# oraclefina/MSPI

Hardware: AMD Instinct MI355X
Metric: clips_per_sec (higher is better)
Workload: dtype f32 storage/accumulate; GEMMs as f16x3 split products on the f16 MFMA pipe; 1 GPU; x3dl motion encoder + ConvNeXt-T + ResNet18 audio + SyncBlock + decoder (AudioVisualSaliencyModel forward), batch 8/GPU, clips 3x16x224x224, spectrogram 1x257x300, inputs resident in HBM; global_batch=8, launch=hipGraph replay (mspi_amd.runtime.GraphPipeline), 2 batches in flight, stream_layout=2, parallelism=single GPU

## Files before the change

include/mspi_hip.h:

```cpp
#ifndef MSPI_HIP_H
#define MSPI_HIP_H

#include <stddef.h>
#include <stdint.h>

#ifdef __cplusplus
extern "C" {
#endif

#define MSPI_ABI_VERSION 2

typedef void* mspi_stream_t;

enum {
  MSPI_OK = 0,
  MSPI_EINVAL = -1,
  MSPI_ELAUNCH = -2,
  MSPI_ENODEV = -3
};

enum { MSPI_ACT_NONE = 0, MSPI_ACT_RELU = 1, MSPI_ACT_GELU = 2, MSPI_ACT_SIGMOID = 3, MSPI_ACT_SWISH = 4 };

enum { MSPI_PREC_F32 = 0, MSPI_PREC_F16X3 = 1 };

// ... 79 lines not shown
int mspi_attn_fwd_ws(const MspiAttnDesc* d, const float* q, const float* k, const float* v, const float* res,
                     const float* biasT, const float* maskT, const int32_t* tok_idx, float* o, void* workspace,
                     mspi_stream_t stream);
int mspi_attn_variant(const MspiAttnDesc* d, int32_t has_bias, int32_t has_mask, int32_t has_tok, int32_t has_ws);

typedef struct MspiMvitAugDesc {
  int32_t B, heads, Dh, DA;
  int32_t qT, qH, qW, kT, kH, kW;
  int64_t ldq, ldk;
  float scale;
} MspiMvitAugDesc;

int mspi_mvit_qk_augment(const MspiMvitAugDesc* d, const float* q, const float* k, const float* Rh, const float* Rw,
                         const float* Rt, float* qa, float* ka, mspi_stream_t stream);

int mspi_mvit_qk_augment_p(const MspiMvitAugDesc* d, const float* q, const float* k, const float* P, int64_t ldp,
                           const int32_t* idx_h, const int32_t* idx_w, const int32_t* idx_t, float* qa, float* ka,
                           mspi_stream_t stream);

typedef struct MspiX3dAbDesc {
  int32_t N, T, H, W;
  int32_t Cin, Cmid;
  int64_t ldx, ldu;
  int32_t act;
  float wa_scale;
} MspiX3dAbDesc;

int mspi_x3d_ab_supported(const MspiX3dAbDesc* d);
int mspi_x3d_ab_pool_rows(const MspiX3dAbDesc* d);
size_t mspi_x3d_ab_packed_bytes(int32_t Cin, int32_t Cmid);
int mspi_x3d_ab_fwd(const MspiX3dAbDesc* d, const void* x, const void* wa_packed, const void* bias_a, const void* wb,
                    const void* bias_b, void* u, void* pool , mspi_stream_t stream);
int mspi_x3d_ab_variant(const MspiX3dAbDesc* d);

int mspi_maxpool_fwd(const MspiDwConvDesc* d, const float* x, float* y, mspi_stream_t stream);

int mspi_upsample_fwd(const float* src, int64_t lds, float* dst, int64_t ldd, int32_t NT, int32_t H,
                      int32_t W, int32_t C, int32_t factor, int32_t accumulate, int32_t act,
                      mspi_stream_t stream);

int mspi_upsample_sum_fwd(const float* const* srcs, const int64_t* lds, const int32_t* factors, int32_t J, float* dst,
                          int64_t ldd, int32_t NT, int32_t Ho, int32_t Wo, int32_t C, int32_t accumulate, int32_t act,
                          mspi_stream_t stream);

int mspi_space_to_depth(const float* x, int64_t ldx, float* y, int64_t ldy, int32_t NT, int32_t H, int32_t W,
                        int32_t C, mspi_stream_t stream);

int mspi_rowgate(float* x, int64_t ldx, const float* mask, int64_t M, int32_t C, mspi_stream_t stream);

int mspi_logsumexp_sub(float* x, int32_t N, int32_t L, mspi_stream_t stream);

int mspi_mean_rows(const float* x, int64_t ldx, int64_t rows_per_sample_stride, float* out, int32_t N,
                   int32_t R, int32_t C, mspi_stream_t stream);

int mspi_mean_rows_slices(int32_t R);
int mspi_mean_rows_ws(const float* x, int64_t ldx, int64_t rows_per_sample_stride, float* out, float* ws, int32_t N,
                      int32_t R, int32_t C, mspi_stream_t stream);

int mspi_neg_cosine(const float* p, const float* z, float* out, int32_t N, int32_t C, float scale,
                    int32_t accumulate, mspi_stream_t stream);

size_t mspi_postprocess_workspace(int32_t N, int32_t H, int32_t W, int32_t Ho, int32_t Wo);
int mspi_postprocess_u8(const float* logmap, unsigned char* out, void* workspace, int32_t N, int32_t H, int32_t W,
                        int32_t Ho, int32_t Wo, mspi_stream_t stream);

typedef struct MspiJpegDesc {
// ... 149 lines not shown
```

mspi_amd/_lib.py:

```python
import ctypes as C
import os

_HERE = os.path.dirname(os.path.abspath(__file__))
LIB_PATH = os.environ.get("MSPI_LIB_PATH") or os.path.join(_HERE, "csrc", "libmspi_hip.so")

ACT_NONE, ACT_RELU, ACT_GELU, ACT_SIGMOID, ACT_SWISH = range(5)
PREC_F32, PREC_F16X3 = 0, 1


class MspiError(RuntimeError):
    pass


class ConvDesc(C.Structure):
    _fields_ = [
        ("N", C.c_int32), ("T", C.c_int32), ("H", C.c_int32), ("W", C.c_int32), ("C", C.c_int32),
        ("sN", C.c_int64), ("sT", C.c_int64), ("sH", C.c_int64), ("sW", C.c_int64), ("sC", C.c_int64),
        ("kT", C.c_int32), ("kH", C.c_int32), ("kW", C.c_int32),
        ("strT", C.c_int32), ("strH", C.c_int32), ("strW", C.c_int32),
        ("padT", C.c_int32), ("padH", C.c_int32), ("padW", C.c_int32),
        ("To", C.c_int32), ("Ho", C.c_int32), ("Wo", C.c_int32),
        ("Cout", C.c_int32),
        ("ldy", C.c_int64), ("ldw", C.c_int64), ("ldr", C.c_int64),
        ("act", C.c_int32),
# ... 38 lines not shown


class MlpDesc(C.Structure):
    _fields_ = [
        ("M", C.c_int64), ("C", C.c_int32), ("hidden", C.c_int32),
        ("ldx", C.c_int64), ("ldr", C.c_int64), ("ldy", C.c_int64),
        ("ln", C.c_int32), ("act", C.c_int32), ("eps", C.c_float),
        ("w1_scale", C.c_float), ("w2_scale", C.c_float),
    ]


class RowGemmDesc(C.Structure):
    _fields_ = [
        ("M", C.c_int64), ("K", C.c_int32), ("N", C.c_int32),
        ("ldx", C.c_int64), ("ldr", C.c_int64), ("ldy", C.c_int64), ("ldg", C.c_int64),
        ("act", C.c_int32), ("rows_per_sample", C.c_int32), ("w_scale", C.c_float),
    ]


class X3dCaDesc(C.Structure):
    _fields_ = [
        ("M", C.c_int64), ("D", C.c_int32), ("Cx", C.c_int32),
        ("ldu", C.c_int64), ("ldr", C.c_int64), ("ldy", C.c_int64), ("ldt", C.c_int64), ("ldg", C.c_int64),
        ("rows_per_sample", C.c_int32), ("wc_scale", C.c_float), ("wa_scale", C.c_float),
    ]


class X3dAbDesc(C.Structure):
    _fields_ = [
        ("N", C.c_int32), ("T", C.c_int32), ("H", C.c_int32), ("W", C.c_int32),
        ("Cin", C.c_int32), ("Cmid", C.c_int32),
        ("ldx", C.c_int64), ("ldu", C.c_int64),
        ("act", C.c_int32), ("wa_scale", C.c_float),
    ]


class PermuteDesc(C.Structure):
    _fields_ = [("dims", C.c_int32 * 6), ("strides", C.c_int64 * 6), ("src_elems", C.c_int64)]


class JpegDesc(C.Structure):
    _fields_ = [
        ("B", C.c_int32), ("H", C.c_int32), ("W", C.c_int32), ("quality", C.c_int32),
        ("pitch", C.c_int64), ("map_stride", C.c_int64), ("file_stride", C.c_int64), ("cap", C.c_int64),
        ("div", C.c_uint16 * 64),
        ("header", C.c_void_p), ("header_len", C.c_int32),
    ]


class JpegDecTables(C.Structure):
    _fields_ = [
        ("scan_len", C.c_int32), ("reserved", C.c_int32),
        ("quant", (C.c_uint16 * 64) * 3),
        ("comp_dc", C.c_uint8 * 4), ("comp_ac", C.c_uint8 * 4),
        ("counts", (C.c_uint8 * 16) * 4),
        ("vals", (C.c_uint8 * 256) * 4),
    ]


class JpegDecInfo(C.Structure):
    _fields_ = [
        ("H", C.c_int32), ("W", C.c_int32), ("ncomp", C.c_int32), ("hs", C.c_int32), ("vs", C.c_int32),
        ("scan_off", C.c_int32), ("scan_len", C.c_int32), ("reserved", C.c_int32),
        ("tables", JpegDecTables),
    ]

# ... 53 lines not shown
    "mspi_logspec_fwd": (C.c_int, [_P, C.c_int64, _P, _P, C.c_int32, _P, _P, C.c_int32, _P]),
    "mspi_resize_norm_fwd": (C.c_int, [_P, C.c_int32, C.c_int32, _P, _P, C.c_int64, C.c_int32, C.c_int32, _P, _P, C.c_int32,
                                        _P, _P, C.c_int32, _P, _P, _P]),
    "mspi_clip_resize_plan": (C.c_int, [_P, C.c_int32, C.c_int32, C.c_int32, C.c_int32, C.c_int32, _P]),
    "mspi_clip_resize_norm_fwd": (C.c_int, [_P, C.c_int32, C.c_int32, C.c_int32, _P, _P, _P, C.c_int32, C.c_int32, C.c_int64,
                                             C.c_int64, C.c_int64, C.c_int64, C.c_int32, C.c_int32, _P, _P, _P, C.c_int32, _P, _P,
                                             _P, C.c_int32, _P, _P, _P]),
    "mspi_layernorm_sp_fwd": (C.c_int, [_P, C.c_int64, C.c_int64, _P, C.c_int64, C.c_int64, _P, _P, C.c_float, C.c_int32,
                                         C.c_int32, C.c_int32, C.c_int32, _P]),
    "mspi_split_planes_fwd": (C.c_int, [_P, C.c_int64, C.c_int64, C.c_int32, _P, C.c_int64, C.c_int64, _P]),
    "mspi_join_planes_fwd": (C.c_int, [_P, C.c_int64, C.c_int64, C.c_int64, C.c_int32, _P, C.c_int64, _P]),
    "mspi_gemm_sp_fwd": (C.c_int, [C.POINTER(ConvDesc), _P, C.c_int64, C.c_int64, _P, _P, _P, _P, _P, C.c_int64, C.c_int64, _P]),
    "mspi_gemm_sp_variant": (C.c_int, [C.POINTER(ConvDesc), _P]),
    "mspi_saliency_metrics": (C.c_int, [_P, _P, _P, _P, C.c_int32, C.c_int32, C.c_int32, _P]),
    "mspi_saliency_auc_ws_bytes": (C.c_size_t, [C.c_int32, C.c_int32]),
    "mspi_saliency_auc_judd": (C.c_int, [_P, C.c_int32, _P, _P, _P, _P, C.c_int32, C.c_int32, _P]),
    "mspi_saliency_sauc_counts": (C.c_int, [_P, _P, _P, _P, C.c_int32, C.c_int32, C.c_int32, _P]),
    "mspi_saliency_ig": (C.c_int, [_P, _P, _P, _P, C.c_int32, C.c_int32, _P]),
    "mspi_resize_bilinear_fwd": (C.c_int, [_P, C.c_int32, _P, C.c_int32, C.c_int32, C.c_int32, C.c_int32, C.c_int32, _P]),
    "mspi_resize_fixation_fwd": (C.c_int, [_P, _P, C.c_int32, C.c_int32, C.c_int32, C.c_int32, C.c_int32, _P]),
    "mspi_rowgemm_packed_bytes": (C.c_size_t, [C.c_int32, C.c_int32]),
    "mspi_rowgemm_supported": (C.c_int, [C.c_int32, C.c_int32]),
    "mspi_rowgemm_fwd": (C.c_int, [C.POINTER(RowGemmDesc), _P, _P, _P, _P, _P, _P, _P]),
    "mspi_rowgemm_variant": (C.c_int, [C.POINTER(RowGemmDesc), C.c_int32]),
    "mspi_x3d_ca_packed_bytes": (C.c_size_t, [C.c_int32, C.c_int32]),
    "mspi_x3d_ca_supported": (C.c_int, [C.c_int32, C.c_int32]),
    "mspi_x3d_ca_fwd": (C.c_int, [C.POINTER(X3dCaDesc), _P, _P, _P, _P, _P, _P, _P, _P, _P]),
    "mspi_x3d_ca_variant": (C.c_int, [C.POINTER(X3dCaDesc), C.c_int32]),
    "mspi_x3d_ab_supported": (C.c_int, [C.POINTER(X3dAbDesc)]),
    "mspi_x3d_ab_pool_rows": (C.c_int, [C.POINTER(X3dAbDesc)]),
    "mspi_x3d_ab_packed_bytes": (C.c_size_t, [C.c_int32, C.c_int32]),
    "mspi_x3d_ab_fwd": (C.c_int, [C.POINTER(X3dAbDesc), _P, _P, _P, _P, _P, _P, _P, _P]),
    "mspi_x3d_ab_variant": (C.c_int, [C.POINTER(X3dAbDesc)]),
    "mspi_mlp_packed_bytes": (C.c_size_t, [C.c_int32, C.c_int32]),
    "mspi_mlp_fwd": (C.c_int, [C.POINTER(MlpDesc), _P, _P, _P, _P, _P, _P, _P, _P, _P]),
    "mspi_mlp_variant": (C.c_int, [C.POINTER(MlpDesc)]),
    "mspi_postprocess_workspace": (C.c_size_t, [C.c_int32, C.c_int32, C.c_int32, C.c_int32, C.c_int32]),
    "mspi_postprocess_u8": (C.c_int, [_P, _P, _P, C.c_int32, C.c_int32, C.c_int32, C.c_int32, C.c_int32, _P]),
    "mspi_jpeg_gray_header": (C.c_int, [C.c_int32, C.c_int32, C.c_int32, _P, C.c_int64]),
    "mspi_jpeg_gray_bound": (C.c_size_t, [C.c_int32, C.c_int32]),
    "mspi_jpeg_gray_ws_bytes": (C.c_size_t, [C.c_int32, C.c_int32, C.c_int32]),
    "mspi_jpeg_gray_fwd": (C.c_int, [C.POINTER(JpegDesc), _P, _P, _P, _P, _P]),
    "mspi_jpeg_dec_parse": (C.c_int, [_P, C.c_int64, C.POINTER(JpegDecInfo)]),
    "mspi_jpeg_dec_ws_bytes": (C.c_size_t, [C.POINTER(JpegDecDesc)]),
    "mspi_jpeg_dec_fwd": (C.c_int, [C.POINTER(JpegDecDesc), _P, _P, _P, _P, _P, _P, _P]),
}

EXPORTS = tuple(_SIGNATURES)

_lib = None


def load():
    global _lib
    if _lib is not None:
        return _lib
    if not os.path.exists(LIB_PATH):
        raise MspiError(
            "libmspi_hip.so not found at %s -- run `python -c 'import __graft_entry__ as g; g.build()'` "
            "(mspi_amd has no CPU fallback)" % LIB_PATH)
    import torch
    lib = C.CDLL(LIB_PATH)
    for name, (res, args) in _SIGNATURES.items():
        fn = getattr(lib, name)
        fn.restype = res
        fn.argtypes = args
# ... 11 lines not shown
```

mspi_amd/backbones/blocks3d.py:

```python
import os

import torch
import torch.nn as nn

from .. import engine as E
from ..module import HipModule


def _t3(v):
    return tuple(v) if isinstance(v, (list, tuple)) else (v, v, v)


class X3DStem(HipModule):

    def __init__(self, dim_in, dim_out, kernel, stride, padding, eps=1e-5, bn_mmt=0.1):
        super().__init__()
        self.kernel, self.stride, self.padding = kernel, stride, padding
        self.conv_xy = nn.Conv3d(dim_in, dim_out, (1, kernel[1], kernel[2]), (1, stride[1], stride[2]),
                                 (0, padding[1], padding[2]), bias=False)
        self.conv = nn.Conv3d(dim_out, dim_out, (kernel[0], 1, 1), (stride[0], 1, 1), (padding[0], 0, 0), bias=False,
                              groups=dim_out)
        self.bn = nn.BatchNorm3d(dim_out, eps=eps, momentum=bn_mmt)
        self.relu = nn.ReLU(True)

    def _pack(self):
        cxy, ct = self.conv_xy, self.conv
        return (E.pack_conv(cxy.weight, None, None, cxy.stride, cxy.padding, E.ACT_NONE),
                E.pack_dwconv(ct.weight, None, self.bn, ct.stride, ct.padding, E.ACT_RELU))

    def run(self, x):
        pxy, pt = self.pk
        return E.dwconv(E.conv(x, pxy), pt)


class ResNetBasicStem(HipModule):

    def __init__(self, dim_in, dim_out, kernel, stride, padding, eps=1e-5, bn_mmt=0.1):
        super().__init__()
        self.conv = nn.Conv3d(dim_in, dim_out, _t3(kernel), _t3(stride), _t3(padding), bias=False)
        self.bn = nn.BatchNorm3d(dim_out, eps=eps, momentum=bn_mmt)
        self.relu = nn.ReLU(True)
        self.pool_layer = nn.MaxPool3d(kernel_size=[1, 3, 3], stride=[1, 2, 2], padding=[0, 1, 1])

    WIDE = 4

    def _pack(self):
        c = self.conv
        pk = {"conv": E.pack_conv(c.weight, None, self.bn, c.stride, c.padding, E.ACT_RELU), "wide": None}
        kw, sw, pw = c.kernel_size[2], c.stride[2], c.padding[2]
        if c.out_channels <= 8 and sw == 2 and kw % 2 == 1 and pw == kw // 2:
            w, b = E.fold_bn(c.weight, None, self.bn)
            G, co = self.WIDE, c.out_channels
            wide = torch.zeros(G * co, w.shape[1], w.shape[2], w.shape[3], kw + (G - 1) * sw, device=w.device)
            for j in range(G):
                wide[j * co:(j + 1) * co, :, :, :, j * sw:j * sw + kw] = w
            pk["wide"] = E.pack_conv(wide, b.repeat(G), None, (c.stride[0], c.stride[1], G * sw), c.padding, E.ACT_RELU)
        return pk

    def run(self, x, out=None):
        pk = self.pk
        W = x.W if isinstance(x, E.CL) else x.shape[-1]
        if pk["wide"] is not None and W % (2 * self.WIDE) == 0:
            y = E.conv(x, pk["wide"])
            y = E.CL(y.buf, y.off, y.N, y.T, y.H, y.W * self.WIDE, self.conv.out_channels, self.conv.out_channels)
# ... 17 lines not shown
        if outs is None:
            return [getattr(self, "pathway{}_stem".format(p)).run(xs[p]) for p in range(self.num_pathways)]
        return [getattr(self, "pathway{}_stem".format(p)).run(xs[p], out=outs[p]) for p in range(self.num_pathways)]


def _se_width(width, ratio, min_width=8, divisor=8):
    if not ratio:
        return width
    width *= ratio
    out = max(min_width, int(width + divisor / 2) // divisor * divisor)
    if out < 0.9 * width:
        out += divisor
    return int(out)


class SE(nn.Module):

    def __init__(self, dim_in, ratio):
        super().__init__()
        dim_fc = _se_width(dim_in, ratio)
        self.avg_pool = nn.AdaptiveAvgPool3d((1, 1, 1))
        self.fc1 = nn.Conv3d(dim_in, dim_fc, 1, bias=True)
        self.fc1_act = nn.ReLU()
        self.fc2 = nn.Conv3d(dim_fc, dim_in, 1, bias=True)
        self.fc2_sig = nn.Sigmoid()


class Swish(nn.Module):
    pass


FUSE_AB = os.environ.get("MSPI_X3D_FUSE", "auto")
FUSE_MIN_W = 56
SEAM = os.environ.get("MSPI_X3D_SEAM", "1")


class X3DTransform(HipModule):
    def __init__(self, dim_in, dim_out, temp_kernel_size, stride, dim_inner, num_groups, stride_1x1=False,
                 eps=1e-5, bn_mmt=0.1, dilation=1, se_ratio=0.0625, swish_inner=True, block_idx=0):
        super().__init__()
        assert num_groups == dim_inner and dilation == 1 and swish_inner, "X3D blocks are channel-wise 3x3x3 + Swish"
        s1, s3 = (stride, 1) if stride_1x1 else (1, stride)
        tk = temp_kernel_size
        self.a = nn.Conv3d(dim_in, dim_inner, (1, 1, 1), (1, s1, s1), 0, bias=False)
        self.a_bn = nn.BatchNorm3d(dim_inner, eps=eps, momentum=bn_mmt)
        self.a_relu = nn.ReLU(True)
        self.b = nn.Conv3d(dim_inner, dim_inner, (tk, 3, 3), (1, s3, s3), (tk // 2, 1, 1), groups=num_groups, bias=False)
        self.b_bn = nn.BatchNorm3d(dim_inner, eps=eps, momentum=bn_mmt)
        if se_ratio > 0.0 and (block_idx + 1) % 2:
            self.se = SE(dim_inner, se_ratio)
        self.b_relu = Swish()
        self.c = nn.Conv3d(dim_inner, dim_out, 1, 1, 0, bias=False)
        self.c_bn = nn.BatchNorm3d(dim_out, eps=eps, momentum=bn_mmt)

    def _pack(self):
        cs_in = E.rup4(self.a.in_channels)
        cs_mid = E.rup4(self.a.out_channels)
        has_se = hasattr(self, "se")
        pk = {
            "a": E.pack_conv(self.a.weight, None, self.a_bn, self.a.stride, (0, 0, 0), E.ACT_RELU, cin_stored=cs_in),
            "b": E.pack_dwconv(self.b.weight, None, self.b_bn, self.b.stride, self.b.padding,
                               E.ACT_NONE if has_se else E.ACT_SWISH),
            "c": E.pack_conv(self.c.weight, None, self.c_bn, (1, 1, 1), (0, 0, 0), E.ACT_RELU, cin_stored=cs_mid),
        }
        pk["ab"] = E.pack_x3d_ab(pk["a"], pk["b"]) if FUSE_AB != "0" else None
        if has_se:
            f, c = self.se.fc1.out_channels, self.se.fc1.in_channels
            dev = self.se.fc1.weight.device
            w1 = torch.zeros(f, cs_mid, device=dev)
            w1[:, :c] = self.se.fc1.weight.detach().float().view(f, c)
            w2 = torch.zeros(cs_mid, f, device=dev)
            w2[:c] = self.se.fc2.weight.detach().float().view(c, f)
            pk["se"] = (w1.contiguous(), self.se.fc1.bias.detach().float().contiguous(), w2.contiguous(),
                        E._pad_vec(self.se.fc2.bias, cs_mid))
        return pk

    def uses_ab(self, x):
        pk = self.pk
        return pk["ab"] is not None and (FUSE_AB == "1" or x.W >= FUSE_MIN_W) and E.x3d_ab_supported(x, pk["ab"])

    def run(self, x, res, out=None, t=None, seam=None):
        pk = self.pk
        se = "se" in pk
        if t is None and self.uses_ab(x) and E.range_check_input(pk["a"], x):
            u = E.x3d_ab(x, pk["ab"], pool=se)
        else:
            u = E.dwconv(E.conv(x, pk["a"]) if t is None else t, pk["b"], pool=se)
        gate = None
        if se:
            u, part = u
            gate = E.se_gate(part, 1.0 / (u.T * u.H * u.W), *pk["se"])
        if seam is not None:
            return E.x3d_ca(u, seam, res, gate=gate)
        return E.conv(u, pk["c"], res=res, gate=gate, out=out)


class BottleneckTransform(HipModule):
    def __init__(self, dim_in, dim_out, temp_kernel_size, stride, dim_inner, num_groups, stride_1x1=False,
                 eps=1e-5, bn_mmt=0.1, dilation=1, block_idx=0):
        super().__init__()
        assert num_groups == 1 and dilation == 1
        s1, s3 = (stride, 1) if stride_1x1 else (1, stride)
        tk = temp_kernel_size
        self.a = nn.Conv3d(dim_in, dim_inner, (tk, 1, 1), (1, s1, s1), (tk // 2, 0, 0), bias=False)
        self.a_bn = nn.BatchNorm3d(dim_inner, eps=eps, momentum=bn_mmt)
        self.a_relu = nn.ReLU(True)
        self.b = nn.Conv3d(dim_inner, dim_inner, (1, 3, 3), (1, s3, s3), (0, 1, 1), bias=False)
        self.b_bn = nn.BatchNorm3d(dim_inner, eps=eps, momentum=bn_mmt)
        self.b_relu = nn.ReLU(True)
        self.c = nn.Conv3d(dim_inner, dim_out, 1, 1, 0, bias=False)
        self.c_bn = nn.BatchNorm3d(dim_out, eps=eps, momentum=bn_mmt)

    def _pack(self):
        return {n: E.pack_conv(c.weight, None, bn, c.stride, c.padding, E.ACT_RELU, cin_stored=E.rup4(c.in_channels))
                for n, c, bn in (("a", self.a, self.a_bn), ("b", self.b, self.b_bn), ("c", self.c, self.c_bn))}

    def run(self, x, res, out=None):
        pk = self.pk
# ... 88 lines not shown
```

mspi_amd/engine.py:

```python
import ctypes as C
import math

import numpy as np
import torch

from . import _lib
from ._lib import (ACT_GELU, ACT_NONE, ACT_RELU, ACT_SIGMOID, ACT_SWISH, PREC_F16X3, PREC_F32, AttnDesc, ConvDesc,
                   DwConvDesc, MspiError, MvitAugDesc, check)

import os as _os
DEFAULT_PREC = {"f32": PREC_F32, "f16x3": PREC_F16X3}[_os.environ.get("MSPI_GEMM_PREC", "f16x3")]

__all__ = ["CL", "SP", "alloc", "alloc_sp", "pack_conv", "pack_dwconv", "PackedConv", "PackedDw", "conv", "dwconv", "maxpool",
           "layernorm", "attention", "upsample", "upsample_sum", "rowgate", "logsumexp_sub", "mean_rows", "neg_cosine",
           "se_gate", "add", "fold_bn", "ACT_NONE", "ACT_RELU", "ACT_GELU", "ACT_SIGMOID", "ACT_SWISH"]


def rup4(c):
    return (c + 3) // 4 * 4


AUTOTUNE = {"on": _os.environ.get("MSPI_AUTOTUNE", "0") == "1", "cache": {}, "reps": 3}


# ... 443 lines not shown
    planes = [pl.view(nch, 2, 16, ks, 4, 8).permute(0, 3, 1, 4, 2, 5).reshape(nch, ks, 2, 64, 8) for pl in (hi, lo)]
    p = PackedX3dAb()
    p.wa = torch.stack(planes, 3).contiguous().to(dev)
    p.ba, p.wb, p.bb = pa.bias, pb.w, pb.bias
    p.wa_scale, p.cin_s, p.cmid, p.cmid_s = pa.w_scale, pa.cin_s, pb.c, pb.c_s
    return p


def _x3d_ab_desc(x, pk, out_ld, act):
    d = _lib.X3dAbDesc()
    d.N, d.T, d.H, d.W = x.N, x.T, x.H, x.W
    d.Cin, d.Cmid, d.ldx, d.ldu, d.act, d.wa_scale = pk.cin_s, pk.cmid_s, x.ld, out_ld, act, pk.wa_scale
    return d


def x3d_ab_supported(x, pk):
    return pk is not None and x.dense and x.Cs == pk.cin_s and bool(_lib.load().mspi_x3d_ab_supported(C.byref(_x3d_ab_desc(x, pk, pk.cmid_s, ACT_NONE))))


def x3d_ab(x, pk, pool=False):
    lib = _lib.load()
    _need_gpu(x.buf)
    out = alloc(x.N, x.T, x.H, x.W, pk.cmid, x.buf.device)
    d = _x3d_ab_desc(x, pk, out.ld, ACT_NONE if pool else ACT_SWISH)
    part = None
    if pool:
        rows = lib.mspi_x3d_ab_pool_rows(C.byref(d))
        part = torch.empty(x.N, rows, pk.cmid_s, dtype=torch.float32, device=x.buf.device)
    with _Timed("x3d_ab_pool" if pool else "x3d_ab", 2.0 * x.M * (pk.cin_s + 27) * pk.cmid, 4.0 * x.M * (x.C + pk.cmid),
                "in=%s Cin=%d Cmid=%d" % ((x.N, x.T, x.H, x.W), x.C, pk.cmid)):
        check(lib.mspi_x3d_ab_fwd(C.byref(d), x.ptr, pk.wa.data_ptr(), pk.ba.data_ptr(), pk.wb.data_ptr(), pk.bb.data_ptr(),
                                  out.ptr, part.data_ptr() if pool else None, _stream()), "mspi_x3d_ab_fwd")
    return (out, part) if pool else out


class PackedX3dCa:
    __slots__ = ("w", "bc", "ba", "d", "cx", "cx_s", "d_s", "wc_scale", "wa_scale")


def x3d_ca_supported(d_s, cx_s):
    return 4 <= d_s <= 224 and d_s % 4 == 0 and 4 <= cx_s <= 256 and cx_s % 4 == 0


def pack_x3d_ca(pc, pa):
    ok = all(q.prec == PREC_F16X3 and q.k == (1, 1, 1) and q.stride == (1, 1, 1) and q.pad == (0, 0, 0) and q.act == ACT_RELU
             and q.bias is not None for q in (pc, pa))
    if not ok or pc.cout_s != pa.cin_s or pc.cin_s != pa.cout_s or not x3d_ca_supported(pc.cin_s, pc.cout_s):
        return None
    d_s, cx_s = pc.cin_s, pc.cout_s
    c = 128 if d_s <= 128 else 224
    hid = (cx_s + 31) // 32 * 32
    nch, ks, ct = hid // 32, c // 16, c // 32
    w1 = torch.zeros(hid, c, dtype=torch.float32)
    w1[:cx_s, :d_s] = (pc.w[0].float() + pc.w[1].float()).cpu()[:, :d_s]
    w2 = torch.zeros(c, hid, dtype=torch.float32)
    w2[:d_s, :cx_s] = (pa.w[0].float() + pa.w[1].float()).cpu()[:, :cx_s]

    def planes(ws):
        hi = ws.to(torch.float16)
        return hi, (ws - hi.float()).to(torch.float16)

    parts1 = [pl.view(nch, 32, ks, 2, 8).permute(0, 2, 3, 1, 4).reshape(nch, ks, 64, 8) for pl in planes(w1)]
    parts2 = [pl.view(ct, 32, nch, 2, 2, 2, 4).permute(2, 3, 0, 5, 1, 4, 6).reshape(nch, 2, ct, 64, 8) for pl in planes(w2)]
    p = PackedX3dCa()
    p.w = torch.cat([torch.stack(parts1, 2).reshape(nch, -1), torch.stack(parts2, 3).reshape(nch, -1)], 1).contiguous().to(pc.w.device)
    p.bc, p.ba = pc.bias, pa.bias
# ... 744 lines not shown
```

Before: 670.8 clips/s.

## Fuse X3D stem convs and stride-2 expand+depthwise into single kernels

Adds a fused X3D stem kernel that computes the spatial 3x3 stride-2 conv and the temporal 5-tap depthwise conv with folded BN and ReLU in one pass, keeping a temporal ring in registers. Adds a stride-2 variant of the fused expand (1x1 f16x3 MFMA) plus 3x3x3 depthwise kernel for the downsampling bottleneck blocks, with an LDS ring over time. Both aim to remove the intermediate activation write/read to HBM and extra launches, at the cost of large register/LDS use and low occupancy (launch_bounds 512,1) and per-call host packing of stem weights into kernel arguments.

```diff
diff --git a/include/mspi_hip.h b/include/mspi_hip.h
--- a/include/mspi_hip.h
+++ b/include/mspi_hip.h
@@ -135,6 +135,31 @@
 int mspi_x3d_ab_fwd(const MspiX3dAbDesc* d, const void* x, const void* wa_packed, const void* bias_a, const void* wb,
                     const void* bias_b, void* u, void* pool , mspi_stream_t stream);
 int mspi_x3d_ab_variant(const MspiX3dAbDesc* d);
+
+typedef struct MspiX3dAbS2Desc {
+  int32_t N, T, H, W;
+  int32_t Cin, Cmid;
+  int64_t ldx, ldu;
+  int32_t act;
+  float wa_scale;
+} MspiX3dAbS2Desc;
+
+int mspi_x3d_ab_s2_supported(const MspiX3dAbS2Desc* d);
+int mspi_x3d_ab_s2_pool_rows(const MspiX3dAbS2Desc* d);
+int mspi_x3d_ab_s2_fwd(const MspiX3dAbS2Desc* d, const void* x, const void* wa_packed, const void* bias_a, const void* wb,
+                       const void* bias_b, void* u, void* pool , mspi_stream_t stream);
+int mspi_x3d_ab_s2_variant(const MspiX3dAbS2Desc* d);
+
+typedef struct MspiX3dStemDesc {
+  int32_t N, T, H, W;
+  int64_t sN, sC, sT, sH, sW;
+  int64_t ldy;
+} MspiX3dStemDesc;
+
+int mspi_x3d_stem_supported(const MspiX3dStemDesc* d);
+int mspi_x3d_stem_variant(const MspiX3dStemDesc* d);
+int mspi_x3d_stem_fwd(const MspiX3dStemDesc* d, const void* x, const void* wxy, const void* wt, const void* bias, void* y,
+                      mspi_stream_t stream);
 
 int mspi_maxpool_fwd(const MspiDwConvDesc* d, const float* x, float* y, mspi_stream_t stream);
 
diff --git a/mspi_amd/_lib.py b/mspi_amd/_lib.py
--- a/mspi_amd/_lib.py
+++ b/mspi_amd/_lib.py
@@ -94,6 +94,18 @@
         ("Cin", C.c_int32), ("Cmid", C.c_int32),
         ("ldx", C.c_int64), ("ldu", C.c_int64),
         ("act", C.c_int32), ("wa_scale", C.c_float),
+    ]
+
+
+class X3dAbS2Desc(C.Structure):
+    _fields_ = list(X3dAbDesc._fields_)
+
+
+class X3dStemDesc(C.Structure):
+    _fields_ = [
+        ("N", C.c_int32), ("T", C.c_int32), ("H", C.c_int32), ("W", C.c_int32),
+        ("sN", C.c_int64), ("sC", C.c_int64), ("sT", C.c_int64), ("sH", C.c_int64), ("sW", C.c_int64),
+        ("ldy", C.c_int64),
     ]
 
 
@@ -213,6 +225,13 @@
     "mspi_x3d_ab_packed_bytes": (C.c_size_t, [C.c_int32, C.c_int32]),
     "mspi_x3d_ab_fwd": (C.c_int, [C.POINTER(X3dAbDesc), _P, _P, _P, _P, _P, _P, _P, _P]),
     "mspi_x3d_ab_variant": (C.c_int, [C.POINTER(X3dAbDesc)]),
+    "mspi_x3d_ab_s2_supported": (C.c_int, [C.POINTER(X3dAbS2Desc)]),
+    "mspi_x3d_ab_s2_pool_rows": (C.c_int, [C.POINTER(X3dAbS2Desc)]),
+    "mspi_x3d_ab_s2_fwd": (C.c_int, [C.POINTER(X3dAbS2Desc), _P, _P, _P, _P, _P, _P, _P, _P]),
+    "mspi_x3d_ab_s2_variant": (C.c_int, [C.POINTER(X3dAbS2Desc)]),
+    "mspi_x3d_stem_supported": (C.c_int, [C.POINTER(X3dStemDesc)]),
+    "mspi_x3d_stem_variant": (C.c_int, [C.POINTER(X3dStemDesc)]),
+    "mspi_x3d_stem_fwd": (C.c_int, [C.POINTER(X3dStemDesc), _P, _P, _P, _P, _P, _P]),
     "mspi_mlp_packed_bytes": (C.c_size_t, [C.c_int32, C.c_int32]),
     "mspi_mlp_fwd": (C.c_int, [C.POINTER(MlpDesc), _P, _P, _P, _P, _P, _P, _P, _P, _P]),
     "mspi_mlp_variant": (C.c_int, [C.POINTER(MlpDesc)]),
diff --git a/mspi_amd/backbones/blocks3d.py b/mspi_amd/backbones/blocks3d.py
--- a/mspi_amd/backbones/blocks3d.py
+++ b/mspi_amd/backbones/blocks3d.py
@@ -5,6 +5,9 @@
 
 from .. import engine as E
 from ..module import HipModule
+
+
+STEM_FUSED = os.environ.get("MSPI_X3D_STEM_FUSED", "1")
 
 
 def _t3(v):
@@ -25,11 +28,17 @@
 
     def _pack(self):
         cxy, ct = self.conv_xy, self.conv
+        fused = None
+        if tuple(cxy.stride) == (1, 2, 2) and tuple(cxy.padding) == (0, 1, 1) and tuple(ct.stride) == (1, 1, 1) \
+                and tuple(ct.padding) == (2, 0, 0):
+            fused = E.pack_x3d_stem(cxy.weight, ct.weight, self.bn)
         return (E.pack_conv(cxy.weight, None, None, cxy.stride, cxy.padding, E.ACT_NONE),
-                E.pack_dwconv(ct.weight, None, self.bn, ct.stride, ct.padding, E.ACT_RELU))
+                E.pack_dwconv(ct.weight, None, self.bn, ct.stride, ct.padding, E.ACT_RELU), fused)
 
     def run(self, x):
-        pxy, pt = self.pk
+        pxy, pt, fused = self.pk
+        if STEM_FUSED != "0" and E.x3d_stem_supported(x, fused):
+            return E.x3d_stem(x, fused)
         return E.dwconv(E.conv(x, pxy), pt)
 
 
@@ -113,6 +122,8 @@
 
 FUSE_AB = os.environ.get("MSPI_X3D_FUSE", "auto")
 FUSE_MIN_W = 56
+FUSE_S2 = os.environ.get("MSPI_X3D_FUSE_S2", "auto")
+FUSE_S2_MIN_W = int(os.environ.get("MSPI_X3D_FUSE_S2_MIN_W", "56"))
 SEAM = os.environ.get("MSPI_X3D_SEAM", "1")
 
 
@@ -145,6 +156,7 @@
             "c": E.pack_conv(self.c.weight, None, self.c_bn, (1, 1, 1), (0, 0, 0), E.ACT_RELU, cin_stored=cs_mid),
         }
         pk["ab"] = E.pack_x3d_ab(pk["a"], pk["b"]) if FUSE_AB != "0" else None
+        pk["ab_s2"] = E.pack_x3d_ab_s2(pk["a"], pk["b"])
         if has_se:
             f, c = self.se.fc1.out_channels, self.se.fc1.in_channels
             dev = self.se.fc1.weight.device
@@ -160,11 +172,18 @@
         pk = self.pk
         return pk["ab"] is not None and (FUSE_AB == "1" or x.W >= FUSE_MIN_W) and E.x3d_ab_supported(x, pk["ab"])
 
+    def uses_ab_s2(self, x):
+        pk = self.pk
+        return pk["ab_s2"] is not None and FUSE_S2 != "0" and (FUSE_S2 == "1" or x.W // 2 >= FUSE_S2_MIN_W) \
+            and E.x3d_ab_s2_supported(x, pk["ab_s2"])
+
     def run(self, x, res, out=None, t=None, seam=None):
         pk = self.pk
         se = "se" in pk
         if t is None and self.uses_ab(x) and E.range_check_input(pk["a"], x):
             u = E.x3d_ab(x, pk["ab"], pool=se)
+        elif t is None and self.uses_ab_s2(x) and E.range_check_input(pk["a"], x):
+            u = E.x3d_ab_s2(x, pk["ab_s2"], pool=se)
         else:
             u = E.dwconv(E.conv(x, pk["a"]) if t is None else t, pk["b"], pool=se)
         gate = None
diff --git a/mspi_amd/csrc/x3d_head.hip b/mspi_amd/csrc/x3d_head.hip
--- /dev/null
+++ b/mspi_amd/csrc/x3d_head.hip
@@ -0,0 +1,423 @@
+#include "conv_common.h"
+#include <stdlib.h>
+#include <string.h>
+
+namespace mspi {
+
+typedef float v4f_s2 __attribute__((ext_vector_type(4)));
+typedef _Float16 v8h_s2 __attribute__((ext_vector_type(8)));
+typedef __attribute__((address_space(3))) void lds_void_s2;
+
+struct X3dAbS2Args {
+  const float* x; const unsigned char* wa; const float* ba; const float* wb; const float* bb; float* u; float* pool;
+  int N, T, H, W, Ho, Wo, Cin, Cmid;
+  long ldx, ldu;
+  int nch, tiles_w, tiles, nseg, tseg;
+  int act;
+  float inv_s;
+  int* status;
+  int dbg;
+};
+
+constexpr int S2_TO = 7;
+constexpr int S2_CH = 2 * S2_TO + 1;
+constexpr int S2_PW = 8;
+constexpr int S2_PLANE = S2_CH * S2_PW;
+constexpr int S2_NCELL = 2 * S2_PLANE;
+constexpr int S2_SLOT = S2_NCELL * 32;
+constexpr int S2_THREADS = 512;
+
+template <int KS>
+__global__ __launch_bounds__(S2_THREADS, 1) void x3d_ab_s2_kernel(const X3dAbS2Args p) {
+  constexpr int NBT = S2_NCELL / 16;
+  constexpr int NW = S2_THREADS / 64;
+  constexpr int MAXT = (NBT + NW - 1) / NW;
+  constexpr int WA_BYTES = KS * 4096;
+  constexpr int NOUT = S2_TO * S2_TO;
+  __shared__ __attribute__((aligned(16))) unsigned char s2_smem[WA_BYTES + 3 * S2_SLOT * 4 + 128];
+  float* ring = reinterpret_cast<float*>(s2_smem + WA_BYTES);
+  float* bias_a = ring + 3 * S2_SLOT;
+
+  const int tid = threadIdx.x, lane = tid & 63, wave = tid >> 6;
+  const int lb = xcd_logical_block((int)blockIdx.x, (int)gridDim.x);
+  const int chunk = lb % p.nch;
+  const int rest = lb / p.nch;
+  const int tile = rest % p.tiles;
+  const int seg = rest / p.tiles;
+  const int n = blockIdx.y;
+  const int h0 = (tile / p.tiles_w) * S2_TO, w0 = (tile % p.tiles_w) * S2_TO;
+  const int t0 = seg * p.tseg;
+  const int tend = min(p.T, t0 + p.tseg);
+
+  for (int i = wave; i < WA_BYTES / 1024; i += NW)
+    __builtin_amdgcn_global_load_lds(reinterpret_cast<const float*>(p.wa + (long)chunk * WA_BYTES + (long)i * 1024 + lane * 16),
+                                     (lds_void_s2*)(s2_smem + i * 1024), 16, 0, 0);
+  if (tid < 32) bias_a[tid] = (chunk * 32 + tid < p.Cmid) ? p.ba[chunk * 32 + tid] : 0.f;
+  const int q = tid & 7;
+  const int cq = chunk * 32 + q * 4;
+  const bool cok = cq < p.Cmid;
+  float4 wreg[27];
+#pragma unroll
+  for (int k = 0; k < 27; ++k) wreg[k] = cok ? *reinterpret_cast<const float4*>(p.wb + (long)k * p.Cmid + cq) : make_float4(0.f, 0.f, 0.f, 0.f);
+  const float4 bq = cok ? *reinterpret_cast<const float4*>(p.bb + cq) : make_float4(0.f, 0.f, 0.f, 0.f);
+  float4 psum = make_float4(0.f, 0.f, 0.f, 0.f);
+  bool bad = false;
+
+  const int li = lane & 15, kg = lane >> 4;
+  int xoff[MAXT];
+#pragma unroll
+  for (int j = 0; j < MAXT; ++j) {
+    const int c = (wave + NW * j) * 16 + li;
+    const int plane = c / S2_PLANE, r = c - plane * S2_PLANE;
+    const int cw = 2 * (r & 7) + plane;
+    const int h = 2 * h0 - 1 + (r >> 3), w = 2 * w0 - 1 + cw;
+    const bool in = c < S2_NCELL && cw < S2_CH && h >= 0 && h < p.H && w >= 0 && w < p.W;
+    xoff[j] = in ? (int)(((long)h * p.W + w) * p.ldx) + 8 * kg : -1;
+  }
+  float4 raw[MAXT][KS][2];
+  auto request = [&](int ta) {
+    const float* xf = p.x + (((long)n * p.T + ta) * p.H) * (long)p.W * p.ldx;
+#pragma unroll
+    for (int j = 0; j < MAXT; ++j)
+#pragma unroll
+      for (int s = 0; s < KS; ++s) {
+        const bool kok = xoff[j] >= 0 && (32 * s + 8 * kg) < p.Cin && !(p.dbg & 4);
+        const float* xr = kok ? xf + xoff[j] + 32 * s : xf;
+        raw[j][s][0] = *reinterpret_cast<const float4*>(xr);
+        raw[j][s][1] = *reinterpret_cast<const float4*>(xr + 4);
+      }
+  };
+  const int nstep = (tend - t0) + 2;
+  if (t0 - 1 >= 0 && !(p.dbg & 1)) request(t0 - 1);
+  asm volatile("s_waitcnt vmcnt(0)" ::: "memory");
+  __syncthreads();
+
+  const int item = tid >> 3;
+  const int oh = item / S2_TO, ow = item - oh * S2_TO;
+#pragma unroll 1
+  for (int i = 0; i < nstep; ++i) {
+    const int ta = t0 - 1 + i;
+    float* slot = ring + (i % 3) * S2_SLOT;
+    if (p.dbg & 1) {
+    } else if (ta < 0 || ta >= p.T) {
+      for (int e = tid * 4; e < S2_SLOT; e += S2_THREADS * 4) *reinterpret_cast<float4*>(slot + e) = make_float4(0.f, 0.f, 0.f, 0.f);
+    } else {
+#pragma unroll
+      for (int j = 0; j < MAXT; ++j) {
+        const int bt = wave + NW * j;
+        if (bt >= NBT) break;
+        const int c = bt * 16 + li;
+        const bool inside = xoff[j] >= 0;
+        v8h_s2 xh[KS], xl[KS];
+#pragma unroll
+        for (int s = 0; s < KS; ++s) {
+          const bool kok = inside && (32 * s + 8 * kg) < p.Cin;
+          const float4 a = raw[j][s][0], b = raw[j][s][1];
+          const float v8[8] = {a.x, a.y, a.z, a.w, b.x, b.y, b.z, b.w};
+#pragma unroll
+          for (int e = 0; e < 8; ++e) {
+            _Float16 hh, ll;
+            split_f16(kok ? v8[e] : 0.f, hh, ll);
+            xh[s][e] = hh; xl[s][e] = ll;
+          }
+        }
+#pragma unroll
+        for (int at = 0; at < 2; ++at) {
+          v4f_s2 acc = {0.f, 0.f, 0.f, 0.f};
+#pragma unroll
+          for (int s = 0; s < KS; ++s) {
+            const unsigned char* wp = s2_smem + ((s * 2 + at) * 2) * 1024 + lane * 16;
+            const v8h_s2 wh = *reinterpret_cast<const v8h_s2*>(wp);
+            const v8h_s2 wl = *reinterpret_cast<const v8h_s2*>(wp + 1024);
+            if (!kSingleProduct) {
+              acc = __builtin_amdgcn_mfma_f32_16x16x32_f16(wl, xh[s], acc, 0, 0, 0);
+              acc = __builtin_amdgcn_mfma_f32_16x16x32_f16(wh, xl[s], acc, 0, 0, 0);
+            }
+            acc = __builtin_amdgcn_mfma_f32_16x16x32_f16(wh, xh[s], acc, 0, 0, 0);
+          }
+          const float4 bv = *reinterpret_cast<const float4*>(bias_a + at * 16 + 4 * kg);
+          bad |= inside && (nonfinite(acc[0]) | nonfinite(acc[1]) | nonfinite(acc[2]) | nonfinite(acc[3]));
+          float4 o;
+          o.x = inside ? fmaxf(fmaf(acc[0], p.inv_s, bv.x), 0.f) : 0.f;
+          o.y = inside ? fmaxf(fmaf(acc[1], p.inv_s, bv.y), 0.f) : 0.f;
+          o.z = inside ? fmaxf(fmaf(acc[2], p.inv_s, bv.z), 0.f) : 0.f;
+          o.w = inside ? fmaxf(fmaf(acc[3], p.inv_s, bv.w), 0.f) : 0.f;
+          *reinterpret_cast<float4*>(slot + c * 32 + (((at * 4 + kg) ^ (c & 3)) << 2)) = o;
+        }
+      }
+    }
+    __syncthreads();
+    if (i + 1 < nstep && ta + 1 >= 0 && ta + 1 < p.T && !(p.dbg & 1)) request(ta + 1);
+    if (i >= 2 && !(p.dbg & 2) && item < NOUT) {
+      const int to = t0 + i - 2;
+      float4 acc = bq;
+#pragma unroll
+      for (int dt = 0; dt < 3; ++dt) {
+        asm volatile("" ::: "memory");
+        const float* sl = ring + ((i - 2 + dt) % 3) * S2_SLOT;
+        float4 win[9];
+#pragma unroll
+        for (int kh = 0; kh < 3; ++kh)
+#pragma unroll
+          for (int kw = 0; kw < 3; ++kw) {
+            const int c = ((kw & 1) * S2_CH + 2 * oh + kh) * S2_PW + ow + (kw >> 1);
+            win[kh * 3 + kw] = *reinterpret_cast<const float4*>(sl + c * 32 + ((q ^ (c & 3)) << 2));
+          }
+#pragma unroll
+        for (int k = 0; k < 9; ++k) {
+          const float4 wv = wreg[dt * 9 + k];
+          acc.x = fmaf(win[k].x, wv.x, acc.x);
+          acc.y = fmaf(win[k].y, wv.y, acc.y);
+          acc.z = fmaf(win[k].z, wv.z, acc.z);
+          acc.w = fmaf(win[k].w, wv.w, acc.w);
+        }
+      }
+      psum.x += acc.x; psum.y += acc.y; psum.z += acc.z; psum.w += acc.w;
+      if (p.act == MSPI_ACT_SWISH) {
+        acc.x = fast_swish(acc.x); acc.y = fast_swish(acc.y); acc.z = fast_swish(acc.z); acc.w = fast_swish(acc.w);
+      }
+      if (cok)
+        *reinterpret_cast<float4*>(p.u + ((((long)n * p.T + to) * p.Ho + (h0 + oh)) * (long)p.Wo + (w0 + ow)) * p.ldu + cq) = acc;
+    }
+    __syncthreads();
+  }
+  report_nonfinite(p.status, bad);
+  if (p.pool) {
+    float* red = ring;
+    *reinterpret_cast<float4*>(red + tid * 4) = psum;
+    __syncthreads();
+    if (tid < 32) {
+      const int qq = tid >> 2, comp = tid & 3;
+      float s = 0.f;
+      for (int r = 0; r < NOUT; ++r) s += red[(r * 8 + qq) * 4 + comp];
+      const int c = chunk * 32 + tid;
+      if (c < p.Cmid) p.pool[((long)n * (p.tiles * p.nseg) + (seg * p.tiles + tile)) * p.Cmid + c] = s;
+    }
+  }
+}
+
+template <int KS>
+static void launch_ab_s2(const X3dAbS2Args& a, hipStream_t s) {
+  const dim3 grid((unsigned)(a.nch * a.tiles * a.nseg), (unsigned)a.N);
+  hipLaunchKernelGGL((x3d_ab_s2_kernel<KS>), grid, dim3(S2_THREADS), 0, s, a);
+}
+
+static int x3d_s2_tseg(int N, int T, int tiles, int nch) {
+  int best = T;
+  for (int ts = T; ts >= 2; ts = (ts + 1) / 2) {
+    best = ts;
+    if ((long)N * tiles * nch * ((T + ts - 1) / ts) >= 448) break;
+    if (ts == 2) break;
+  }
+  return best;
+}
+
+static void x3d_s2_geometry(const MspiX3dAbS2Desc* d, X3dAbS2Args& a) {
+  a.Ho = d->H / 2; a.Wo = d->W / 2;
+  a.nch = (d->Cmid + 31) / 32;
+  a.tiles_w = a.Wo / S2_TO;
+  a.tiles = (a.Ho / S2_TO) * a.tiles_w;
+  a.tseg = x3d_s2_tseg(d->N, d->T, a.tiles, a.nch);
+  a.nseg = (d->T + a.tseg - 1) / a.tseg;
+}
+
+
+constexpr int STEM_C = 24;
+
+struct X3dStemArgs {
+  const float* x; float* y;
+  float wxy[STEM_C][28], wt[STEM_C][8];
+  int N, T, H, W, Ho, Wo;
+  long sN, sC, sT, sH, sW, ldy;
+  int tseg, nseg;
+};
+
+__global__ __launch_bounds__(256) void x3d_stem_kernel(const X3dStemArgs p) {
+  const int npix = p.Ho * p.Wo;
+  const int pix0 = blockIdx.x * 256 + threadIdx.x;
+  const bool live = pix0 < npix;
+  const int pix = live ? pix0 : 0;
+  const int ho = pix / p.Wo, wo = pix - ho * p.Wo;
+  const int n = blockIdx.z;
+  const int t0 = blockIdx.y * p.tseg;
+  const int tend = min(p.T, t0 + p.tseg);
+  int off[9];
+  unsigned ok = 0;
+#pragma unroll
+  for (int kh = 0; kh < 3; ++kh)
+#pragma unroll
+    for (int kw = 0; kw < 3; ++kw) {
+      const int h = 2 * ho - 1 + kh, w = 2 * wo - 1 + kw;
+      const bool in = h >= 0 && h < p.H && w >= 0 && w < p.W;
+      off[kh * 3 + kw] = in ? (int)(h * p.sH + w * p.sW) : 0;
+      ok |= (in ? 1u : 0u) << (kh * 3 + kw);
+    }
+  const float* xn = p.x + (long)n * p.sN;
+  float nxt[27];
+  auto request = [&](int f) {
+    const float* xf = xn + (long)f * p.sT;
+#pragma unroll
+    for (int ci = 0; ci < 3; ++ci)
+#pragma unroll
+      for (int k = 0; k < 9; ++k) nxt[ci * 9 + k] = xf[ci * p.sC + off[k]];
+  };
+  float ring[5][STEM_C];
+#pragma unroll
+  for (int j = 0; j < 5; ++j)
+#pragma unroll
+    for (int c = 0; c < STEM_C; ++c) ring[j][c] = 0.f;
+  const int nstep = (tend - t0) + 4;
+  if (t0 - 2 >= 0) request(t0 - 2);
+#pragma unroll 1
+  for (int i = 0; i < nstep; ++i) {
+    const int f = t0 - 2 + i;
+    int z = 0;
+    asm volatile("" : "+s"(z));
+#pragma unroll
+    for (int j = 0; j < 4; ++j)
+#pragma unroll
+      for (int c = 0; c < STEM_C; ++c) ring[j][c] = ring[j + 1][c];
+    if (f >= 0 && f < p.T) {
+      float cur[27];
+#pragma unroll
+      for (int k = 0; k < 27; ++k) cur[k] = ((ok >> (k % 9)) & 1u) ? nxt[k] : 0.f;
+      if (i + 1 < nstep && f + 1 < p.T) request(f + 1);
+#pragma unroll
+      for (int c = 0; c < STEM_C; ++c) {
+        float a = 0.f;
+#pragma unroll
+        for (int k = 0; k < 27; ++k) a = fmaf(cur[k], p.wxy[c][z + k], a);
+        ring[4][c] = a;
+      }
+    } else {
+      if (i + 1 < nstep && f + 1 >= 0 && f + 1 < p.T) request(f + 1);
+#pragma unroll
+      for (int c = 0; c < STEM_C; ++c) ring[4][c] = 0.f;
+    }
+    if (i >= 4) {
+      const int to = f - 2;
+      float* yp = p.y + ((((long)n * p.T + to) * p.Ho + ho) * (long)p.Wo + wo) * p.ldy;
+#pragma unroll
+      for (int c4 = 0; c4 < STEM_C; c4 += 4) {
+        float o[4];
+#pragma unroll
+        for (int e = 0; e < 4; ++e) {
+          const int c = c4 + e;
+          float a = p.wt[c][z + 5];
+#pragma unroll
+          for (int k = 0; k < 5; ++k) a = fmaf(ring[k][c], p.wt[c][z + k], a);
+          o[e] = fmaxf(a, 0.f);
+        }
+        if (live) *reinterpret_cast<float4*>(yp + c4) = make_float4(o[0], o[1], o[2], o[3]);
+      }
+    }
+  }
+}
+
+static int x3d_stem_tseg(const MspiX3dStemDesc* d) {
+  const int ho = (d->H - 1) / 2 + 1, wo = (d->W - 1) / 2 + 1;
+  const long waves = (long)d->N * ((ho * wo + 255) / 256) * 4;
+  int ts = d->T;
+  while (ts > 4 && waves * ((d->T + ts - 1) / ts) < 1024) ts = (ts + 1) / 2;
+  return ts;
+}
+
+}
+
+using namespace mspi;
+
+extern "C" int mspi_x3d_ab_s2_supported(const MspiX3dAbS2Desc* d) {
+  if (!d) return 0;
+  if (d->H < 2 || d->W < 2 || d->H % 2 || d->W % 2 || d->T < 1) return 0;
+  const int ks = (d->Cin + 31) / 32;
+  const bool tile_ok = (d->H / 2) % S2_TO == 0 && (d->W / 2) % S2_TO == 0;
+  return ks >= 1 && ks <= 3 && tile_ok && d->Cin % 8 == 0 && d->Cmid % 4 == 0 && d->Cin >= 8 && d->Cmid >= 4;
+}
+
+extern "C" int mspi_x3d_ab_s2_pool_rows(const MspiX3dAbS2Desc* d) {
+  if (!mspi_x3d_ab_s2_supported(d)) return 0;
+  X3dAbS2Args a;
+  x3d_s2_geometry(d, a);
+  return a.tiles * a.nseg;
+}
+
+static int x3d_ab_s2_select(const MspiX3dAbS2Desc* d) {
+  MSPI_REQUIRE(mspi_x3d_ab_s2_supported(d), "mspi_x3d_ab_s2_fwd: shape N=%d T=%d H=%d W=%d Cin=%d Cmid=%d is outside the fused kernel's range",
+               d->N, d->T, d->H, d->W, d->Cin, d->Cmid);
+  MSPI_REQUIRE(d->N >= 1 && d->N < 65536 && d->ldx >= d->Cin && d->ldu >= d->Cmid && d->ldx % 4 == 0 && d->ldu % 4 == 0,
+               "mspi_x3d_ab_s2_fwd: row strides must cover the row and be multiples of 4 floats");
+  MSPI_REQUIRE((long)d->H * d->W * d->ldx < (1L << 31), "mspi_x3d_ab_s2_fwd: one frame of x must stay below 2^31 floats");
+  MSPI_REQUIRE(d->act == MSPI_ACT_NONE || d->act == MSPI_ACT_SWISH, "mspi_x3d_ab_s2_fwd: act must be NONE or SWISH");
+  MSPI_REQUIRE(d->wa_scale > 0.f, "mspi_x3d_ab_s2_fwd: wa_scale must be positive");
+  return ((d->Cin + 31) / 32) * 10000 + 7071;
+}
+
+extern "C" int mspi_x3d_ab_s2_variant(const MspiX3dAbS2Desc* d) {
+  MSPI_REQUIRE(d, "mspi_x3d_ab_s2_variant: null descriptor");
+  return x3d_ab_s2_select(d);
+}
+
+extern "C" int mspi_x3d_ab_s2_fwd(const MspiX3dAbS2Desc* d, const void* x, const void* wa_packed, const void* bias_a, const void* wb,
+                                  const void* bias_b, void* u, void* pool, void* stream) {
+  MSPI_REQUIRE(d && x && wa_packed && bias_a && wb && bias_b && u, "mspi_x3d_ab_s2_fwd: null argument");
+  const int variant = x3d_ab_s2_select(d);
+  if (variant < 0) return variant;
+  MSPI_REQUIRE(aligned16(x) && aligned16(u) && aligned16(wb) && aligned16(bias_b) && aligned16(wa_packed), "mspi_x3d_ab_s2_fwd: 16-byte alignment");
+  X3dAbS2Args a;
+  a.x = (const float*)x; a.wa = (const unsigned char*)wa_packed; a.ba = (const float*)bias_a; a.wb = (const float*)wb;
+  a.bb = (const float*)bias_b; a.u = (float*)u; a.pool = (float*)pool;
+  a.N = d->N; a.T = d->T; a.H = d->H; a.W = d->W; a.Cin = d->Cin; a.Cmid = d->Cmid; a.ldx = d->ldx; a.ldu = d->ldu;
+  a.act = d->act; a.inv_s = 1.0f / d->wa_scale;
+  static const int dbg = getenv("MSPI_X3D_DBG") ? atoi(getenv("MSPI_X3D_DBG")) : 0;
+  static const int tseg_env = getenv("MSPI_X3D_TSEG") ? atoi(getenv("MSPI_X3D_TSEG")) : 0;
+  a.dbg = dbg;
+  a.status = g_status_word;
+  x3d_s2_geometry(d, a);
+  if (tseg_env > 0 && !pool) { a.tseg = tseg_env; a.nseg = (d->T + a.tseg - 1) / a.tseg; }
+  hipStream_t s = (hipStream_t)stream;
+  switch (variant / 10000) {
+    case 1: launch_ab_s2<1>(a, s); break;
+    case 2: launch_ab_s2<2>(a, s); break;
+    default: launch_ab_s2<3>(a, s); break;
+  }
+  return check_launch("mspi_x3d_ab_s2_fwd");
+}
+
+
+extern "C" int mspi_x3d_stem_supported(const MspiX3dStemDesc* d) {
+  if (!d) return 0;
+  if (d->N < 1 || d->N >= 65536 || d->T < 1 || d->T >= 65536 || d->H < 1 || d->W < 1) return 0;
+  if (d->sN < 0 || d->sC < 0 || d->sT < 0 || d->sH < 0 || d->sW < 0) return 0;
+  return (long)(d->H - 1) * d->sH + (long)(d->W - 1) * d->sW < (1L << 31) && (long)d->H * d->W < (1L << 31);
+}
+
+extern "C" int mspi_x3d_stem_variant(const MspiX3dStemDesc* d) {
+  MSPI_REQUIRE(d, "mspi_x3d_stem_variant: null descriptor");
+  MSPI_REQUIRE(mspi_x3d_stem_supported(d), "mspi_x3d_stem_fwd: shape N=%d T=%d H=%d W=%d or its strides are outside the fused stem's range",
+               d->N, d->T, d->H, d->W);
+  return x3d_stem_tseg(d);
+}
+
+extern "C" int mspi_x3d_stem_fwd(const MspiX3dStemDesc* d, const void* x, const void* wxy, const void* wt, const void* bias, void* y,
+                                 void* stream) {
+  MSPI_REQUIRE(d && x && wxy && wt && bias && y, "mspi_x3d_stem_fwd: null argument");
+  const int tseg = mspi_x3d_stem_variant(d);
+  if (tseg < 0) return tseg;
+  MSPI_REQUIRE(d->ldy >= STEM_C && d->ldy % 4 == 0, "mspi_x3d_stem_fwd: the output row stride must cover 24 channels and be a multiple of 4 floats");
+  MSPI_REQUIRE(aligned16(y) && (reinterpret_cast<uintptr_t>(x) & 3u) == 0, "mspi_x3d_stem_fwd: y must be 16-byte aligned, x 4-byte aligned");
+  X3dStemArgs a;
+  a.x = (const float*)x; a.y = (float*)y;
+  const float *hxy = (const float*)wxy, *ht = (const float*)wt, *hb = (const float*)bias;
+  memset(a.wxy, 0, sizeof(a.wxy)); memset(a.wt, 0, sizeof(a.wt));
+  for (int c = 0; c < STEM_C; ++c) {
+    for (int k = 0; k < 27; ++k) a.wxy[c][k] = hxy[k * STEM_C + c];
+    for (int k = 0; k < 5; ++k) a.wt[c][k] = ht[k * STEM_C + c];
+    a.wt[c][5] = hb[c];
+  }
+  a.N = d->N; a.T = d->T; a.H = d->H; a.W = d->W; a.Ho = (d->H - 1) / 2 + 1; a.Wo = (d->W - 1) / 2 + 1;
+  a.sN = d->sN; a.sC = d->sC; a.sT = d->sT; a.sH = d->sH; a.sW = d->sW; a.ldy = d->ldy;
+  a.tseg = tseg; a.nseg = (d->T + tseg - 1) / tseg;
+  const dim3 grid((unsigned)((a.Ho * a.Wo + 255) / 256), (unsigned)a.nseg, (unsigned)a.N);
+  hipLaunchKernelGGL(x3d_stem_kernel, grid, dim3(256), 0, (hipStream_t)stream, a);
+  return check_launch("mspi_x3d_stem_fwd");
+}
diff --git a/mspi_amd/engine.py b/mspi_amd/engine.py
--- a/mspi_amd/engine.py
+++ b/mspi_amd/engine.py
@@ -499,6 +499,95 @@
         check(lib.mspi_x3d_ab_fwd(C.byref(d), x.ptr, pk.wa.data_ptr(), pk.ba.data_ptr(), pk.wb.data_ptr(), pk.bb.data_ptr(),
                                   out.ptr, part.data_ptr() if pool else None, _stream()), "mspi_x3d_ab_fwd")
     return (out, part) if pool else out
+
+
+def pack_x3d_ab_s2(pa, pb):
+    if pb.stride != (1, 2, 2) or (pa.cin_s + 31) // 32 > 3:
+        return None
+    s1 = PackedDw()
+    for f in PackedDw.__slots__:
+        setattr(s1, f, getattr(pb, f))
+    s1.stride = (1, 1, 1)
+    return pack_x3d_ab(pa, s1)
+
+
+def _x3d_ab_s2_desc(x, pk, out_ld, act):
+    d = _lib.X3dAbS2Desc()
+    d.N, d.T, d.H, d.W = x.N, x.T, x.H, x.W
+    d.Cin, d.Cmid, d.ldx, d.ldu, d.act, d.wa_scale = pk.cin_s, pk.cmid_s, x.ld, out_ld, act, pk.wa_scale
+    return d
+
+
+def x3d_ab_s2_supported(x, pk):
+    return pk is not None and x.dense and x.Cs == pk.cin_s \
+        and bool(_lib.load().mspi_x3d_ab_s2_supported(C.byref(_x3d_ab_s2_desc(x, pk, pk.cmid_s, ACT_NONE))))
+
+
+def x3d_ab_s2(x, pk, pool=False, out=None):
+    lib = _lib.load()
+    _need_gpu(x.buf)
+    if not x3d_ab_s2_supported(x, pk):
+        raise MspiError("x3d_ab_s2: input %s with %d channels is outside the fused kernel's range" % ((x.N, x.T, x.H, x.W), x.C))
+    if out is None:
+        out = alloc(x.N, x.T, x.H // 2, x.W // 2, pk.cmid, x.buf.device)
+    elif (out.N, out.T, out.H, out.W, out.Cs) != (x.N, x.T, x.H // 2, x.W // 2, pk.cmid_s) or not out.dense:
+        raise MspiError("x3d_ab_s2: the output tensor does not match the layer")
+    d = _x3d_ab_s2_desc(x, pk, out.ld, ACT_NONE if pool else ACT_SWISH)
+    part = None
+    if pool:
+        rows = lib.mspi_x3d_ab_s2_pool_rows(C.byref(d))
+        part = torch.empty(x.N, rows, pk.cmid_s, dtype=torch.float32, device=x.buf.device)
+    with _Timed("x3d_ab_s2_pool" if pool else "x3d_ab_s2", 2.0 * x.M * pk.cin_s * pk.cmid + 2.0 * out.M * 27 * pk.cmid,
+                4.0 * (x.M * x.C + out.M * pk.cmid), "in=%s Cin=%d Cmid=%d" % ((x.N, x.T, x.H, x.W), x.C, pk.cmid)):
+        check(lib.mspi_x3d_ab_s2_fwd(C.byref(d), x.ptr, pk.wa.data_ptr(), pk.ba.data_ptr(), pk.wb.data_ptr(), pk.bb.data_ptr(),
+                                     out.ptr, part.data_ptr() if pool else None, _stream()), "mspi_x3d_ab_s2_fwd")
+    return (out, part) if pool else out
+
+
+class PackedX3dStem:
+    __slots__ = ("wxy", "wt", "bias")
+
+
+def pack_x3d_stem(w_xy, w_t, bn):
+    if tuple(w_xy.shape) != (24, 3, 1, 3, 3) or tuple(w_t.shape) != (24, 1, 5, 1, 1):
+        return None
+    wt, b = fold_bn(w_t, None, bn)
+    p = PackedX3dStem()
+    p.wxy = w_xy.detach().float().cpu().reshape(24, 27).t().contiguous()
+    p.wt = wt.detach().float().cpu().reshape(24, 5).t().contiguous()
+    p.bias = (b if b is not None else torch.zeros(24)).detach().float().cpu().contiguous()
+    return p
+
+
+def _x3d_stem_desc(x, ldy):
+    d = _lib.X3dStemDesc()
+    d.N, _, d.T, d.H, d.W = x.shape
+    d.sN, d.sC, d.sT, d.sH, d.sW = x.stride()
+    d.ldy = ldy
+    return d
+
+
+def x3d_stem_supported(x, pk):
+    return pk is not None and isinstance(x, torch.Tensor) and x.dim() == 5 and x.shape[1] == 3 and x.dtype == torch.float32 \
+        and x.data_ptr() % 4 == 0 and bool(_lib.load().mspi_x3d_stem_supported(C.byref(_x3d_stem_desc(x, 24))))
+
+
+def x3d_stem(x, pk, out=None):
+    lib = _lib.load()
+    _need_gpu(x)
+    if not x3d_stem_supported(x, pk):
+        raise MspiError("x3d_stem: input %s is outside the fused stem's range" % (tuple(x.shape),))
+    N, _, T, H, W = x.shape
+    Ho, Wo = (H - 1) // 2 + 1, (W - 1) // 2 + 1
+    if out is None:
+        out = alloc(N, T, Ho, Wo, 24, x.device)
+    elif (out.N, out.T, out.H, out.W, out.Cs) != (N, T, Ho, Wo, 24) or not out.dense:
+        raise MspiError("x3d_stem: the output tensor does not match the layer")
+    d = _x3d_stem_desc(x, out.ld)
+    with _Timed("x3d_stem", 2.0 * out.M * 24 * (27 + 5), 4.0 * (N * 3 * T * H * W + out.M * 24), "in=%s" % (tuple(x.shape),)):
+        check(lib.mspi_x3d_stem_fwd(C.byref(d), x.data_ptr(), pk.wxy.data_ptr(), pk.wt.data_ptr(), pk.bias.data_ptr(), out.ptr,
+                                    _stream()), "mspi_x3d_stem_fwd")
+    return out
 
 
 class PackedX3dCa:
```

Measured after the change: 684.8 clips/s, median of 6. 1.02x the previous value.
